# Tangshitao/Semi-supervised-Adaptive-Distillation

Hardware: AMD Instinct MI355X
Metric: images/sec (student+teacher fwd + student bwd) R50-FPN distill, 1/2/4/8 MI355X (higher is better)
Workload: dtype f32

## Files before the change

### include/ssad_kernels.h

```cpp
#ifndef SSAD_KERNELS_H_
#define SSAD_KERNELS_H_

#include <stddef.h>
#include <stdint.h>

#ifdef __cplusplus
extern "C" {
#endif

#define SSAD_API __attribute__((visibility("default")))

#define SSAD_E_BADARG (-1)
#define SSAD_E_WORKSPACE (-2)
#define SSAD_MAX_LEVELS 8
#define SSAD_MAX_CONV_PROBLEMS 24
#define SSAD_MAX_POWSUM_INPUTS 8

typedef void* ssad_stream_t;


typedef struct {
  float gamma;
  float alpha;
  float beta;
// ... 225 lines not shown
                         float* col, ssad_stream_t stream);
SSAD_API int ssad_im2col_batched(const float* x, int N, int C, int H, int W, int kernel, int stride,
                                 int pad, float* col, ssad_stream_t stream);
SSAD_API int ssad_col2im(const float* col, int C, int H, int W, int kh, int kw, int dil_h,
                         int dil_w, int pad_t, int pad_l, int pad_b, int pad_r, int stride_h,
                         int stride_w, float* x, ssad_stream_t stream);
SSAD_API int ssad_channel_sum(const float* dy, int N, int C, int HW, float* out, int accumulate,
                              ssad_stream_t stream);
SSAD_API int ssad_relu_grad_rowsum(const float* y, const float* dy, float* dx, float* rowsum, int N,
                                   int C, int HW, ssad_stream_t stream);
SSAD_API int ssad_conv1x1_bias_act(const float* x, const float* w, const float* bias,
                                   const float* residual, float* y, int N, int C, int P, int M,
                                   int relu, ssad_stream_t stream);
SSAD_API int ssad_conv1x1_bias_act2(const float* x, int C1, const float* x2, int C2, const float* w,
                                    const float* bias, const float* residual, float* y, int N, int P,
                                    int M, int relu, ssad_stream_t stream);
#define SSAD_GEMM_RELU 1
#define SSAD_GEMM_ACCUMULATE 8
typedef struct ssad_gemm_conv {
  const float* a;
  const float* x;
  float* y;
  const float* bias;
  const float* residual;
  const float* mask;
  int lda, N, K, P, M, flags;
} ssad_gemm_conv;
SSAD_API int ssad_conv1x1_gemm(const ssad_gemm_conv* desc_host, ssad_stream_t stream);
SSAD_API size_t ssad_conv1x1_gemm_split_workspace_bytes(const ssad_gemm_conv* desc_host);
SSAD_API int ssad_conv1x1_gemm_split(const ssad_gemm_conv* desc_host, void* workspace, size_t workspace_bytes,
                                     ssad_stream_t stream);
SSAD_API int ssad_conv1x1_gemm_split_amax(const ssad_gemm_conv* desc_host, const float* packed_a, const unsigned* x_amax,
                                          unsigned* y_amax_out, void* workspace, size_t workspace_bytes,
                                          ssad_stream_t stream);
typedef struct ssad_gemm_pack_entry {
  const float* a;
  float* dst;
  int lda, K, M;
} ssad_gemm_pack_entry;
SSAD_API size_t ssad_gemm_split_filter_floats(int K, int M);
SSAD_API int ssad_gemm_split_pack_filters(const ssad_gemm_pack_entry* entries_host, int n_entries, ssad_stream_t stream);
SSAD_API int ssad_conv_implicit_gemm(const ssad_gemm_conv* d, int C, int H, int W, int kernel, int stride, int pad,
                                     ssad_stream_t stream);
SSAD_API size_t ssad_conv_implicit_gemm_workspace_bytes(int N, int M, int C, int H, int W, int kernel, int stride,
                                                        int pad);
SSAD_API int ssad_conv_implicit_gemm_ws(const ssad_gemm_conv* d, int C, int H, int W, int kernel, int stride, int pad,
                                        void* workspace, size_t workspace_bytes, ssad_stream_t stream);
SSAD_API size_t ssad_conv_kxk_wgrad_workspace_bytes(int N, int C, int H, int W, int M, int kernel, int stride,
                                                    int pad);
SSAD_API int ssad_conv_kxk_wgrad(const float* x, const float* dy, int N, int C, int H, int W, int M, int kernel,
                                 int stride, int pad, float* dw, int accumulate, void* workspace,
                                 size_t workspace_bytes, ssad_stream_t stream);
SSAD_API size_t ssad_conv_kxk_dgrad_workspace_bytes(int N, int C, int H, int W, int M, int kernel, int stride,
                                                    int pad);
SSAD_API int ssad_conv_kxk_dgrad(const float* w, const float* dy, int N, int C, int H, int W, int M, int kernel,
                                 int stride, int pad, float* dx, const float* mask, int accumulate, void* workspace,
                                 size_t workspace_bytes, ssad_stream_t stream);
SSAD_API int ssad_transpose_filter(const float* w, int M, int K, int ldm, float* wt, ssad_stream_t stream);
#define SSAD_MAX_TRANSPOSE_ENTRIES 64
typedef struct ssad_transpose_entry {
  const float* w;
  float* wt;
  int M, K, ldm;
  int reserved;
} ssad_transpose_entry;
SSAD_API int ssad_transpose_filters(const ssad_transpose_entry* entries_host, int n_entries, ssad_stream_t stream);
// ... 146 lines not shown
```

### semi-supervised-adaptive-distillation_amd/csrc/kernels/gemm_split.hip

```cpp
#include <stdlib.h>

#include <mutex>

#include "split_common.h"

namespace {

using namespace ssad_split;

constexpr int PT = 128;
constexpr int MT = 256;
constexpr int HDR = 16;

__host__ __device__ constexpr int cdiv(int a, int b) { return (a + b - 1) / b; }

__global__ __launch_bounds__(kThreads) void gsplit_pack_a_kernel(const float* __restrict__ a, int lda, int K, int M,
                                                                 const unsigned* __restrict__ amax, float* __restrict__ dst) {
  const int KB = (K + 7) >> 3;
  const long long slots = (long long)KB * M;
  const float s = pow2f(15 - split_exponent(amax[0]));
  if (blockIdx.x == 0 && threadIdx.x < HDR) reinterpret_cast<unsigned*>(dst)[threadIdx.x] = threadIdx.x == 0 ? amax[0] : 0u;
  uint4* out = reinterpret_cast<uint4*>(dst + HDR);
  for (long long i = (long long)blockIdx.x * kThreads + threadIdx.x; i < slots; i += (long long)gridDim.x * kThreads) {
    const int m = (int)(i % M), kb = (int)(i / M);
    float v[8];
#pragma unroll
    for (int j = 0; j < 8; ++j) v[j] = kb * 8 + j < K ? a[(long long)(kb * 8 + j) * lda + m] : 0.0f;
    half8 hi, lo;
    split8(v, s, hi, lo);
    out[i] = __builtin_bit_cast(uint4, hi);
    out[slots + i] = __builtin_bit_cast(uint4, lo);
  }
}

struct GPackTable {
  ssad_gemm_pack_entry e[SSAD_MAX_PACK_ENTRIES];
  int count;
};
__global__ __launch_bounds__(kThreads) void gsplit_zero_kernel(const GPackTable t) {
  for (int i = (int)threadIdx.x; i < t.count * HDR; i += kThreads) reinterpret_cast<unsigned*>(t.e[i / HDR].dst)[i % HDR] = 0u;
}
__global__ __launch_bounds__(kThreads) void gsplit_amax_kernel(const GPackTable t) {
  const ssad_gemm_pack_entry& E = t.e[blockIdx.y];
// ... 9 lines not shown
    m = m > other ? m : other;
  }
  __shared__ unsigned red[kThreads / 64];
  if ((threadIdx.x & 63) == 0) red[threadIdx.x >> 6] = m;
  __syncthreads();
  if (threadIdx.x == 0) {
    for (int w = 1; w < kThreads / 64; ++w) m = m > red[w] ? m : red[w];
    if (m) atomicMax(reinterpret_cast<unsigned*>(E.dst), m);
  }
}
__global__ __launch_bounds__(kThreads) void gsplit_pack_multi_kernel(const GPackTable t) {
  const ssad_gemm_pack_entry& E = t.e[blockIdx.y];
  const int KB = (E.K + 7) >> 3;
  const long long slots = (long long)KB * E.M;
  const float s = pow2f(15 - split_exponent(reinterpret_cast<const unsigned*>(E.dst)[0]));
  uint4* out = reinterpret_cast<uint4*>(E.dst + HDR);
  for (long long i = (long long)blockIdx.x * kThreads + threadIdx.x; i < slots; i += (long long)gridDim.x * kThreads) {
    const int m = (int)(i % E.M), kb = (int)(i / E.M);
    float v[8];
#pragma unroll
    for (int j = 0; j < 8; ++j) v[j] = kb * 8 + j < E.K ? E.a[(long long)(kb * 8 + j) * E.lda + m] : 0.0f;
    half8 hi, lo;
    split8(v, s, hi, lo);
    out[i] = __builtin_bit_cast(uint4, hi);
    out[slots + i] = __builtin_bit_cast(uint4, lo);
  }
}

#ifndef GFLY_ABLATE
#define GFLY_ABLATE 0
#endif
constexpr int FKC = 32;
constexpr int FWG = 512;
constexpr int F_XP = (FKC / 8) * PT * 16;
constexpr int F_WP = (FKC / 8) * MT * 16;
constexpr int F_STAGE = 2 * F_XP + 2 * F_WP;
constexpr int F_LDS = 2 * F_STAGE;

struct FArgs {
  const float* x;
  const float* ap;
  float* y;
  const float* bias;
  const float* residual;
  const float* mask;
  const unsigned* amax;
  unsigned* amax_out;
  int N, K, P, M, relu, accumulate;
  int ptiles, mblocks, items;
};

__global__ __launch_bounds__(FWG, 1) void gemm_fly_kernel(const FArgs q) {
  extern __shared__ __attribute__((aligned(16))) char flds[];
  const int tid = threadIdx.x, lane = tid & 63;
  const int wave = __builtin_amdgcn_readfirstlane(tid >> 6);
  const int wm = wave & 3, wp = wave >> 2;
  const int j = lane & 31, h = lane >> 5;
  const int K = q.K, M = q.M, P = q.P;
  const int KB = (K + 7) >> 3;
  const int nchunks = (K + FKC - 1) / FKC;

  int n, p0, ocb;
  {
    const int it = (int)blockIdx.x;
    const int xcd = it & 7, seq = it >> 3;
    const int mb = seq % q.mblocks;
    const int t = (seq / q.mblocks) * 8 + xcd;
    if (t >= q.N * q.ptiles) return;
    n = t / q.ptiles;
    p0 = (t - n * q.ptiles) * PT;
    ocb = mb * MT;
  }
  const unsigned w_lo_off = (unsigned)((long long)KB * M * 16);
  const __amdgpu_buffer_rsrc_t xrs = uniform_rsrc(q.x, (unsigned)((long long)q.N * K * P * 4));
  const __amdgpu_buffer_rsrc_t wrs = uniform_rsrc(q.ap + HDR, 2u * w_lo_off);
  const float sx = pow2f(15 - split_exponent(q.amax[0]));

  float xv[8];
  f32x4 wv[4];
  const int fpx = tid & (PT - 1), fkg = tid >> 7;
  const int fco = tid & (MT - 1), fkq = tid >> 8;
  const unsigned xbase = p0 + fpx < P ? (unsigned)((((long long)n * K + 8 * fkg) * P + p0 + fpx) * 4) : kOob;
  const int P4 = P * 4;
  auto fetch = [&](int c) {
    const int soff = __builtin_amdgcn_readfirstlane(c * FKC * P4);
#pragma unroll
    for (int e = 0; e < 8; ++e)
      xv[e] = __builtin_bit_cast(float, __builtin_amdgcn_raw_buffer_load_b32(
          xrs, c * FKC + 8 * fkg + e < K ? xbase : kOob, soff + e * P4, 0));
#pragma unroll
    for (int i = 0; i < 2; ++i) {
      const int kb = c * (FKC / 8) + fkq + 2 * i;
      const unsigned vo = (kb < KB && ocb + fco < M) ? (unsigned)((kb * M + ocb + fco) * 16) : kOob;
      wv[2 * i] = __builtin_bit_cast(f32x4, __builtin_amdgcn_raw_buffer_load_b128(wrs, vo, 0, 0));
      wv[2 * i + 1] = __builtin_bit_cast(f32x4, __builtin_amdgcn_raw_buffer_load_b128(wrs, vo, (int)w_lo_off, 0));
    }
  };
  auto put = [&](char* stage) {
    half8 hi, lo;
    split8(xv, sx, hi, lo);
    char* px = stage + (fkg * PT + fpx) * 16;
    *reinterpret_cast<half8*>(px) = hi;
    *reinterpret_cast<half8*>(px + F_XP) = lo;
#pragma unroll
    for (int i = 0; i < 2; ++i) {
      char* pw = stage + 2 * F_XP + ((fkq + 2 * i) * MT + fco) * 16;
      *reinterpret_cast<f32x4*>(pw) = wv[2 * i];
      *reinterpret_cast<f32x4*>(pw + F_WP) = wv[2 * i + 1];
    }
  };

  float16v acc[2][2];
#pragma unroll
  for (int i = 0; i < 2; ++i)
#pragma unroll
    for (int tt = 0; tt < 2; ++tt)
#pragma unroll
      for (int r = 0; r < 16; ++r) acc[i][tt][r] = 0.0f;

  auto step = [&](const char* stage, int st) {
    half8 ah[2], al[2], bh[2], bl[2];
    const int kg = 2 * st + h;
#pragma unroll
    for (int i = 0; i < 2; ++i) {
      const char* pw = stage + 2 * F_XP + (kg * MT + wm * 64 + i * 32 + j) * 16;
      ah[i] = *reinterpret_cast<const half8*>(pw);
      al[i] = *reinterpret_cast<const half8*>(pw + F_WP);
      const char* px = stage + (kg * PT + wp * 64 + i * 32 + j) * 16;
      bh[i] = *reinterpret_cast<const half8*>(px);
      bl[i] = *reinterpret_cast<const half8*>(px + F_XP);
    }
#pragma unroll
    for (int pr = 0; pr < ((GFLY_ABLATE & 8) ? 0 : (GFLY_ABLATE & 4) ? 1 : 3); ++pr)
#pragma unroll
      for (int i = 0; i < 2; ++i)
#pragma unroll
        for (int tt = 0; tt < 2; ++tt)
          acc[i][tt] = __builtin_amdgcn_mfma_f32_32x32x16_f16(pr == 1 ? al[i] : ah[i], pr == 2 ? bl[tt] : bh[tt],
                                                              acc[i][tt], 0, 0, 0);
    if (GFLY_ABLATE & 8) {
#pragma unroll
      for (int i = 0; i < 2; ++i) { acc[i][0][0] += (float)ah[i][0] + (float)al[i][1]; acc[i][1][0] += (float)bh[i][0] + (float)bl[i][1]; }
    }
  };

  fetch(0);
  put(flds);
  fetch(1);
  __syncthreads();
  for (int c = 0; c < nchunks; ++c) {
    const char* stage = flds + (c & 1) * F_STAGE;
    char* other = flds + ((c & 1) ^ 1) * F_STAGE;
    __builtin_amdgcn_sched_barrier(0);
    step(stage, 0);
    if (!(GFLY_ABLATE & 2)) put(other);
    __builtin_amdgcn_sched_barrier(0);
    if (!(GFLY_ABLATE & 1)) fetch(c + 2);
    __builtin_amdgcn_sched_barrier(0);
    step(stage, 1);
    __syncthreads();
  }

  const int oc_w = ocb + wm * 64;
  unsigned pvo[2];
#pragma unroll
  for (int tt = 0; tt < 2; ++tt) {
    const int px = p0 + wp * 64 + 32 * tt + j;
    pvo[tt] = px < P ? (unsigned)((((long long)n * M + 4 * h) * P + px) * 4) : kOob;
  }
  const int e2 = split_exponent(q.amax[0]) + split_exponent(reinterpret_cast<const unsigned*>(q.ap)[0]) - 30;
  const bool one_scale = e2 >= -126 && e2 <= 127;
  const float sc1 = one_scale ? pow2f(e2) : pow2f(split_exponent(q.amax[0]) - 15);
  const float sc2 = one_scale ? 1.0f : pow2f(split_exponent(reinterpret_cast<const unsigned*>(q.ap)[0]) - 15);
  const unsigned ybytes = (unsigned)((long long)q.N * M * P * 4);
  const __amdgpu_buffer_rsrc_t yrs = uniform_rsrc(q.y, ybytes);
  const __amdgpu_buffer_rsrc_t rrs = uniform_rsrc(q.residual ? (const void*)q.residual : (const void*)q.y, q.residual ? ybytes : 0u);
  const __amdgpu_buffer_rsrc_t mrs = uniform_rsrc(q.mask ? (const void*)q.mask : (const void*)q.y, q.mask ? ybytes : 0u);
  const __amdgpu_buffer_rsrc_t brs = uniform_rsrc(q.bias ? (const void*)q.bias : (const void*)q.y, q.bias ? (unsigned)M * 4u : 0u);
  const bool relu = q.relu, has_res = q.residual != nullptr, has_mask = q.mask != nullptr, accum = q.accumulate;
  const bool ragged = (M & 7) != 0;
  unsigned ymax = 0;
#pragma unroll
  for (int i = 0; i < 2; ++i) {
    const int oc0 = oc_w + i * 32;
    float4 bq[4];
#pragma unroll
    for (int g = 0; g < 4; ++g)
      bq[g] = __builtin_bit_cast(float4, __builtin_amdgcn_raw_buffer_load_b128(brs, (unsigned)h * 16u, (oc0 + 8 * g) * 4, 0));
#pragma unroll
    for (int tt = 0; tt < 2; ++tt) {
      float rs[16], mk[16], old[16];
#pragma unroll
      for (int r = 0; r < 16; ++r) {
        const int ch = oc0 + 8 * (r >> 2) + (r & 3);
        const unsigned vo = (ch < M && (!ragged || ch + 4 * h < M)) ? pvo[tt] : kOob;
        rs[r] = has_res ? __builtin_bit_cast(float, __builtin_amdgcn_raw_buffer_load_b32(rrs, vo, ch * P4, 0)) : 0.0f;
        mk[r] = has_mask ? __builtin_bit_cast(float, __builtin_amdgcn_raw_buffer_load_b32(mrs, vo, ch * P4, 0)) : 1.0f;
        old[r] = accum ? __builtin_bit_cast(float, __builtin_amdgcn_raw_buffer_load_b32(yrs, vo, ch * P4, 0)) : 0.0f;
      }
#pragma unroll
      for (int g = 0; g < 4; ++g) {
        if (oc0 + 8 * g >= M) continue;
#pragma unroll
        for (int e = 0; e < 4; ++e) {
          const int r = 4 * g + e;
          float v = one_scale ? fmaf(acc[i][tt][r], sc1, bq[g][e]) : acc[i][tt][r] * sc1 * sc2 + bq[g][e];
          v += rs[r];
          if (relu) v = fmaxf(v, 0.0f);
          if (has_mask) v = mk[r] > 0.0f ? v : 0.0f;
          v += old[r];
          const unsigned vo = (!ragged || oc0 + 8 * g + 4 * h + e < M) ? pvo[tt] : kOob;
          __builtin_amdgcn_raw_buffer_store_b32(__builtin_bit_cast(unsigned, v), yrs, vo, (oc0 + 8 * g + e) * P4, 0);
          const unsigned av = __builtin_bit_cast(unsigned, v) & 0x7fffffffu;
          if (vo != kOob) ymax = ymax > av ? ymax : av;
        }
      }
    }
  }
  if (q.amax_out) {
#pragma unroll
    for (int o = 32; o > 0; o >>= 1) {
      const unsigned other = (unsigned)__shfl_xor((int)ymax, o, 64);
      ymax = ymax > other ? ymax : other;
    }
    __syncthreads();
    unsigned* red = reinterpret_cast<unsigned*>(flds);
    if (lane == 0) red[wave] = ymax;
    __syncthreads();
    if (tid == 0) {
      for (int w = 1; w < FWG / 64; ++w) ymax = ymax > red[w] ? ymax : red[w];
      if (ymax) atomicMax(q.amax_out, ymax);
    }
  }
}

constexpr int WT = 256;
constexpr int WPX = 32;
constexpr int W_PL = (WPX / 8) * WT * 16;
constexpr int W_STAGE = 4 * W_PL;
constexpr int W_LDS = 2 * W_STAGE;

struct WPArgs {
  const float* x;
  const float* dy;
  float* slabs;
  const unsigned* xa;
  const unsigned* da;
  int N, C, P, M;
  int mtiles, ctiles, shares, per_share, total, cpi;
  int xcd_runs;
};

__global__ __launch_bounds__(FWG, 1) void wpoint_split_kernel(const WPArgs q) {
  extern __shared__ __attribute__((aligned(16))) char wlds[];
  const int tid = threadIdx.x, lane = tid & 63;
  const int wave = __builtin_amdgcn_readfirstlane(tid >> 6);
  const int wm = wave & 1, wc = wave >> 1;
  const int j = lane & 31, h = lane >> 5;
  const int P = q.P;

  const int tiles = q.mtiles * q.ctiles;
  int share, tile;
  if (q.xcd_runs) {
// ... 119 lines not shown
__global__ __launch_bounds__(256) void wpoint_reduce_kernel(const float* __restrict__ slabs, int shares, int Mp, int Cp,
                                                            int M, int C, const unsigned* __restrict__ xa,
                                                            const unsigned* __restrict__ da,
                                                            float* __restrict__ dw, int accumulate) {
  const long long e = (long long)blockIdx.x * 256 + threadIdx.x;
  if (e >= (long long)M * C) return;
  const int m = (int)(e / C), c = (int)(e - (long long)m * C);
  const float* p = slabs + (long long)m * Cp + c;
  const long long stride = (long long)Mp * Cp;
  float s = 0.0f;
  for (int sh = 0; sh < shares; ++sh) s += p[sh * stride];
  s = (s * pow2f(split_exponent(xa[0]) - 15)) * pow2f(split_exponent(da[0]) - 15);
  dw[e] = accumulate ? dw[e] + s : s;
}

int wpoint_plan(int N, int C, int P, int M, WPArgs* a) {
  if (N <= 0 || C <= 0 || P <= 0 || M <= 0 || (P & 7)) return SSAD_E_BADARG;
  if ((long long)N * C * P * 4 >= (1LL << 31) || (long long)N * M * P * 4 >= (1LL << 31)) return SSAD_E_BADARG;
  a->N = N; a->C = C; a->P = P; a->M = M;
  a->mtiles = cdiv(M, WT); a->ctiles = cdiv(C, WT);
  a->cpi = cdiv(P, WPX);
  a->total = N * a->cpi;
  const int cus = ssad_cu_count(), tiles = a->mtiles * a->ctiles;
  int s = cus / tiles;
  if (s < 1) s = 1;
  if (s >= 8) s &= ~7;
  while (s > 1 && a->total / s < 4) --s;
  a->per_share = cdiv(a->total, s);
  a->shares = cdiv(a->total, a->per_share);
  a->xcd_runs = (a->shares % 8 == 0) ? a->shares / 8 : 0;
  return 0;
}

struct GPlan {
  size_t amax_off, a_off, total;
};
int make_plan(const ssad_gemm_conv* d, GPlan* p) {
  if (!d || d->N <= 0 || d->K <= 0 || d->P <= 0 || d->M <= 0 || d->lda < d->M) return SSAD_E_BADARG;
  const int KB = (d->K + 7) >> 3;
  const long long aslots = (long long)KB * d->M;
  if ((long long)d->N * d->K * d->P * 4 >= (1LL << 31) || (long long)d->N * d->M * d->P * 4 >= (1LL << 31) ||
      aslots * 32 >= (1LL << 31))
    return SSAD_E_BADARG;
  p->amax_off = 0;
  p->a_off = 256;
  p->total = p->a_off + (size_t)HDR * 4 + (size_t)aslots * 32;
  return 0;
}

}

extern "C" {

size_t ssad_conv1x1_gemm_split_workspace_bytes(const ssad_gemm_conv* d) {
  GPlan p;
  return make_plan(d, &p) ? 0 : p.total;
}

size_t ssad_gemm_split_filter_floats(int K, int M) {
  if (K <= 0 || M <= 0) return 0;
  return (size_t)HDR + (size_t)((K + 7) >> 3) * M * 8;
}

int ssad_gemm_split_pack_filters(const ssad_gemm_pack_entry* entries_host, int n_entries, ssad_stream_t stream_) {
  hipStream_t stream = (hipStream_t)stream_;
  if (!entries_host || n_entries < 0) return SSAD_E_BADARG;
  for (int base = 0; base < n_entries; base += SSAD_MAX_PACK_ENTRIES) {
    GPackTable t;
    const int cnt = n_entries - base < SSAD_MAX_PACK_ENTRIES ? n_entries - base : SSAD_MAX_PACK_ENTRIES;
    long long most = 0;
    for (int i = 0; i < cnt; ++i) {
      t.e[i] = entries_host[base + i];
      if (!t.e[i].a || !t.e[i].dst || t.e[i].K <= 0 || t.e[i].M <= 0 || t.e[i].lda < t.e[i].M) return SSAD_E_BADARG;
      const long long slots = (long long)((t.e[i].K + 7) >> 3) * t.e[i].M;
      if (slots > most) most = slots;
    }
    t.count = cnt;
    hipLaunchKernelGGL(gsplit_zero_kernel, dim3(1), dim3(kThreads), 0, stream, t);
    hipLaunchKernelGGL(gsplit_amax_kernel, dim3(64u, (unsigned)cnt), dim3(kThreads), 0, stream, t);
    long long bx = (most + kThreads - 1) / kThreads;
    if (bx > 256) bx = 256;
    hipLaunchKernelGGL(gsplit_pack_multi_kernel, dim3((unsigned)bx, (unsigned)cnt), dim3(kThreads), 0, stream, t);
  }
  return (int)hipGetLastError();
}

int ssad_conv1x1_gemm_split(const ssad_gemm_conv* d, void* workspace, size_t workspace_bytes, ssad_stream_t stream_) {
  return ssad_conv1x1_gemm_split_amax(d, nullptr, nullptr, nullptr, workspace, workspace_bytes, stream_);
}

int ssad_conv1x1_gemm_split_amax(const ssad_gemm_conv* d, const float* packed_a, const unsigned* x_amax,
                                 unsigned* y_amax_out, void* workspace, size_t workspace_bytes, ssad_stream_t stream_) {
  hipStream_t stream = (hipStream_t)stream_;
  GPlan p;
  const int rc = make_plan(d, &p);
  if (rc) return rc;
  if (!d->a || !d->x || !d->y) return SSAD_E_BADARG;
  if ((d->flags & SSAD_GEMM_ACCUMULATE) && (d->bias || d->residual)) return SSAD_E_BADARG;
  if (!workspace || workspace_bytes < p.total) return SSAD_E_WORKSPACE;
  char* ws = (char*)workspace;
  unsigned* amax = (unsigned*)(ws + p.amax_off);
  float* apk = (float*)(ws + p.a_off);
  const int KB = (d->K + 7) >> 3;
  AmaxTable at;
  for (int l = 0; l < kMaxLv; ++l) { at.x[l] = nullptr; at.n[l] = 0; at.block_start[l] = 0; }
  at.count = 2;
  at.amax = amax;
  at.x[0] = d->x; at.n[0] = (long long)d->N * d->K * d->P;
  at.x[1] = d->a; at.n[1] = (long long)d->K * d->lda;
  int blocks = 0;
  for (int l = 0; l < 2; ++l) {
    at.block_start[l] = blocks;
    long long nb = (at.n[l] / 4 + kThreads * 32 - 1) / (kThreads * 32);
    blocks += (int)(nb < 1 ? 1 : nb > 512 ? 512 : nb);
  }
  for (int l = 2; l <= kMaxLv; ++l) at.block_start[l] = blocks;
  if (x_amax && packed_a) {
  } else {
    if (x_amax) { at.n[0] = 0; }
    if (packed_a) { at.n[1] = 0; }
    (void)hipMemsetAsync(amax, 0, 256, stream);
    hipLaunchKernelGGL(split_absmax_kernel, dim3((unsigned)blocks), dim3(kThreads), 0, stream, at);
    if (!packed_a) {
      long long bx = ((long long)KB * d->M + kThreads - 1) / kThreads;
      if (bx > 1024) bx = 1024;
      hipLaunchKernelGGL(gsplit_pack_a_kernel, dim3((unsigned)bx), dim3(kThreads), 0, stream, d->a, d->lda, d->K, d->M,
                         (const unsigned*)(amax + 1), apk);
    }
  }
  FArgs f;
  f.x = d->x; f.ap = packed_a ? packed_a : apk; f.y = d->y; f.bias = d->bias; f.residual = d->residual; f.mask = d->mask;
  f.amax = x_amax ? x_amax : amax;
  f.amax_out = y_amax_out;
  f.N = d->N; f.K = d->K; f.P = d->P; f.M = d->M;
  f.relu = (d->flags & SSAD_GEMM_RELU) ? 1 : 0;
  f.accumulate = (d->flags & SSAD_GEMM_ACCUMULATE) ? 1 : 0;
  f.ptiles = cdiv(d->P, PT);
  f.mblocks = cdiv(d->M, MT);
  const long long tiles = (long long)d->N * f.ptiles;
  if (tiles * f.mblocks >= (1LL << 30)) return SSAD_E_BADARG;
  f.items = (int)(cdiv((int)tiles, 8) * 8 * f.mblocks);
  static std::once_flag lds_once;
  std::call_once(lds_once, [&] {
    (void)hipFuncSetAttribute((const void*)gemm_fly_kernel, hipFuncAttributeMaxDynamicSharedMemorySize, F_LDS);
  });
  hipLaunchKernelGGL(gemm_fly_kernel, dim3((unsigned)f.items), dim3(FWG), F_LDS, stream, f);
  return (int)hipGetLastError();
}

int ssad_split_absmax(const float* x, long long n, unsigned* word, ssad_stream_t stream_) {
  if (!x || !word || n <= 0) return SSAD_E_BADARG;
  AmaxTable at;
  for (int l = 0; l < kMaxLv; ++l) { at.x[l] = nullptr; at.n[l] = 0; at.block_start[l] = 0; }
  at.count = 1;
  at.amax = word;
  at.x[0] = x; at.n[0] = n;
  long long nb = (n / 4 + kThreads * 32 - 1) / (kThreads * 32);
  const int blocks = (int)(nb < 1 ? 1 : nb > 512 ? 512 : nb);
  for (int l = 1; l <= kMaxLv; ++l) at.block_start[l] = blocks;
  hipLaunchKernelGGL(split_absmax_kernel, dim3((unsigned)blocks), dim3(kThreads), 0, (hipStream_t)stream_, at);
  return (int)hipGetLastError();
}

size_t ssad_conv1x1_wgrad_split_workspace_bytes(int N, int C, int P, int M) {
  WPArgs a;
  if (wpoint_plan(N, C, P, M, &a)) return 0;
  return 256 + sizeof(float) * (size_t)a.shares * a.mtiles * WT * a.ctiles * WT;
}

int ssad_conv1x1_wgrad_split(const float* x, const float* dy, int N, int C, int P, int M, float* dw, int accumulate,
                             void* workspace, size_t workspace_bytes, ssad_stream_t stream_) {
  return ssad_conv1x1_wgrad_split_amax(x, dy, N, C, P, M, dw, accumulate, workspace, workspace_bytes, nullptr, nullptr,
                                       stream_);
}

int ssad_conv1x1_wgrad_split_amax(const float* x, const float* dy, int N, int C, int P, int M, float* dw, int accumulate,
                                  void* workspace, size_t workspace_bytes, const unsigned* x_amax,
                                  const unsigned* dy_amax, ssad_stream_t stream_) {
  hipStream_t stream = (hipStream_t)stream_;
  if ((x_amax == nullptr) != (dy_amax == nullptr)) return SSAD_E_BADARG;
// ... 41 lines not shown
```

### semi-supervised-adaptive-distillation_amd/kernels.py

```python
import ctypes as C
import os

import torch

_HERE = os.path.dirname(os.path.abspath(__file__))
LIB_NAME = "libcaffe2_detectron_ops_hip.so"
LIB_PATH = os.path.join(_HERE, LIB_NAME)

MAX_LEVELS = 8
CONV_RELU = 1
CONV_MASK_AUX = 2
CONV_SIGMOID = 4
CONV_SPLIT_TAIL = 8


class KernelError(RuntimeError):
    pass


class DistillParams(C.Structure):
    _fields_ = [("gamma", C.c_float), ("alpha", C.c_float), ("beta", C.c_float),
                ("num_classes", C.c_int), ("ignored_label", C.c_int),
                ("scale", C.c_float)]

# ... 150 lines not shown
    L.ssad_conv_wino_pack_filter.argtypes = [vp, i32, i32, vp, vp, vp]
    L.ssad_conv3x3_forward_wino.argtypes = [C.POINTER(ConvLevel), i32, vp, vp, i32, i32, i32, vp]
    L.ssad_conv3x3_forward_wino24.argtypes = [C.POINTER(ConvLevel), i32, vp, vp, i32, i32, i32, vp]
    L.ssad_conv_wino24_filter_floats.restype = sz
    L.ssad_conv_wino24_filter_floats.argtypes = [i32, i32]
    L.ssad_conv_wino24_pack_filters.argtypes = [C.POINTER(PackEntry), i32, vp]
    L.ssad_conv_split_filter_floats.restype = sz
    L.ssad_conv_split_filter_floats.argtypes = [i32, i32]
    L.ssad_conv_split_pack_filters.argtypes = [C.POINTER(PackEntry), i32, vp]
    L.ssad_conv3x3_split_workspace_bytes.restype = sz
    L.ssad_conv3x3_split_workspace_bytes.argtypes = [C.POINTER(ConvLevel), i32, i32]
    L.ssad_conv3x3_forward_split.argtypes = [C.POINTER(ConvLevel), i32, vp, vp, i32, i32, i32, vp, sz, vp, vp, vp]
    L.ssad_conv3x3_forward_wino_launches.argtypes = [C.POINTER(ConvLevel), i32]
    L.ssad_conv3x3_forward_wino_launches_for.argtypes = [C.POINTER(ConvLevel), i32, i32, i32, i32]
    L.ssad_conv_wino_split_tail.argtypes = [i32]
    L.ssad_conv3x3_wgrad_workspace_bytes.restype = sz
    L.ssad_conv3x3_wgrad_workspace_bytes.argtypes = [C.POINTER(ConvLevel), i32, i32, i32]
    L.ssad_conv3x3_wgrad.argtypes = [C.POINTER(ConvLevel), i32, vp, vp, i32, i32, i32, vp, sz, vp]
    L.ssad_conv3x3_wgrad_split_workspace_bytes.restype = sz
    L.ssad_conv3x3_wgrad_split_workspace_bytes.argtypes = [C.POINTER(ConvLevel), i32, i32, i32]
    L.ssad_conv3x3_wgrad_split.argtypes = [C.POINTER(ConvLevel), i32, vp, vp, i32, i32, i32, vp, sz, vp]
    L.ssad_conv1x1_gemm.argtypes = [C.POINTER(GemmConv), vp]
    L.ssad_conv1x1_gemm_split_workspace_bytes.restype = sz
    L.ssad_conv1x1_gemm_split_workspace_bytes.argtypes = [C.POINTER(GemmConv)]
    L.ssad_conv1x1_gemm_split.argtypes = [C.POINTER(GemmConv), vp, sz, vp]
    L.ssad_transpose_filter.argtypes = [vp, i32, i32, i32, vp, vp]
    L.ssad_conv1x1_wgrad_workspace_bytes.restype = sz
    L.ssad_conv1x1_wgrad_workspace_bytes.argtypes = [i32, i32, i32, i32]
    L.ssad_conv1x1_wgrad.argtypes = [vp, vp, i32, i32, i32, i32, vp, i32, vp, sz, vp]
    L.ssad_gemm_split_filter_floats.restype = sz
    L.ssad_gemm_split_filter_floats.argtypes = [i32, i32]
    L.ssad_gemm_split_pack_filters.argtypes = [C.POINTER(GemmPackEntry), i32, vp]
    L.ssad_conv1x1_gemm_split_amax.argtypes = [vp, vp, vp, vp, vp, sz, vp]
    L.ssad_split_absmax.argtypes = [vp, C.c_longlong, vp, vp]
    L.ssad_split_absmax_levels.argtypes = [C.POINTER(ConvLevel), i32, i32, i32, vp, vp]
    L.ssad_conv3x3_wgrad_split_amax.argtypes = [C.POINTER(ConvLevel), i32, vp, vp, i32, i32, i32, vp, sz, vp, vp, vp]
    L.ssad_conv1x1_wgrad_split_amax.argtypes = [vp, vp, i32, i32, i32, i32, vp, i32, vp, sz, vp, vp, vp]
    L.ssad_conv1x1_wgrad_split_workspace_bytes.restype = sz
    L.ssad_conv1x1_wgrad_split_workspace_bytes.argtypes = [i32, i32, i32, i32]
    L.ssad_conv1x1_wgrad_split.argtypes = [vp, vp, i32, i32, i32, i32, vp, i32, vp, sz, vp]
    L.ssad_subsample.argtypes = [vp, i32, i32, i32, i32, i32, vp, vp]
    L.ssad_subsample_grad.argtypes = [vp, i32, i32, i32, i32, i32, i32, vp, vp]
    L.ssad_conv_implicit_gemm.argtypes = [C.POINTER(GemmConv), i32, i32, i32, i32, i32, i32, vp]
    L.ssad_transpose_filters.argtypes = [C.POINTER(TransposeEntry), i32, vp]
    L.ssad_f16_pack_filters.argtypes = [C.POINTER(F16PackEntry), i32, vp]
    L.ssad_conv_implicit_gemm_workspace_bytes.restype = sz
    L.ssad_conv_implicit_gemm_workspace_bytes.argtypes = [i32] * 8
    L.ssad_conv_implicit_gemm_ws.argtypes = [C.POINTER(GemmConv), i32, i32, i32, i32, i32, i32, vp, sz, vp]
    L.ssad_conv_kxk_wgrad_workspace_bytes.restype = sz
    L.ssad_conv_kxk_wgrad_workspace_bytes.argtypes = [i32] * 8
    L.ssad_conv_kxk_wgrad.argtypes = [vp, vp, i32, i32, i32, i32, i32, i32, i32, i32, vp, i32, vp, sz, vp]
    L.ssad_conv_kxk_dgrad_workspace_bytes.restype = sz
    L.ssad_conv_kxk_dgrad_workspace_bytes.argtypes = [i32] * 8
    L.ssad_conv_kxk_dgrad.argtypes = [vp, vp, i32, i32, i32, i32, i32, i32, i32, i32, vp, vp, i32, vp, sz, vp]
    L.ssad_grouped_conv3x3_forward.argtypes = [vp, vp, vp, i32, i32, i32, i32, i32, i32, i32, vp, vp]
    L.ssad_grouped_conv3x3_filter_floats.argtypes = [i32, i32]
    L.ssad_grouped_conv3x3_filter_floats.restype = C.c_longlong
    L.ssad_grouped_conv3x3_pack_filter.argtypes = [vp, i32, i32, vp, vp]
    L.ssad_conv1x1_f16.argtypes = [C.POINTER(PwF16), vp]
    L.ssad_pw_f16_filter_halves.restype = sz
    L.ssad_pw_f16_filter_halves.argtypes = [i32, i32]
    L.ssad_pw_f16_pack_filter.argtypes = [vp, i32, i32, vp, vp, vp]
    L.ssad_conv1x1_wgrad_f16_workspace_bytes.restype = sz
    L.ssad_conv1x1_wgrad_f16_workspace_bytes.argtypes = [i32, i32, i32, i32, i32]
    L.ssad_conv1x1_wgrad_f16.argtypes = [vp, vp, i32, i32, i32, i32, i32, i32, f32, vp, vp, vp, vp, sz, vp]
    L.ssad_f16_elementwise.argtypes = [i32, vp, vp, vp, i32, i32, i32, i32, i32, i32, vp]
# ... 612 lines not shown
            arr[i].packed = p["packed"].data_ptr()
            arr[i].bias = p["bias"].data_ptr() if p.get("bias") is not None else None
            i += 1
    flags = ((CONV_RELU if relu else 0) | (CONV_SIGMOID if sigmoid else 0)
             | (CONV_MASK_AUX if masked[0] else 0) | (F16_OUT_NCHW_F32 if out_nchw_f32 else 0))
    _check(lib().ssad_conv3x3_forward_f16_levels(arr, n, None, None, Cin, Cout, flags, _stream()),
           "conv3x3_forward_f16_multi")


def conv3x3_wgrad_f16(xbs, dybs, Cin, Cout, *, scale=1.0, dW=None, db=None, bias_grad=True):
    if dW is None:
        dW = torch.empty((Cout, Cin, 3, 3), dtype=torch.float32, device="cuda")
    if db is None and bias_grad:
        db = torch.empty((Cout,), dtype=torch.float32, device="cuda")
    L = lib()
    n = len(xbs)
    arr = (F16WgradLevel * n)()
    for i, (xb, dyb) in enumerate(zip(xbs, dybs)):
        N, CB, H, W, _ = xb.shape
        assert xb.dtype == torch.float16 and dyb.dtype == torch.float16
        assert xb.is_contiguous() and dyb.is_contiguous()
        assert CB == (Cin + 7) // 8 and dyb.shape == (N, (Cout + 7) // 8, H, W, 8)
        arr[i].x, arr[i].dy, arr[i].N, arr[i].H, arr[i].W = xb.data_ptr(), dyb.data_ptr(), N, H, W
    nbytes = L.ssad_conv3x3_wgrad_f16_levels_workspace_bytes(arr, n, Cin, Cout)
    ws = _workspace(nbytes, "wgrad_f16")
    _check(L.ssad_conv3x3_wgrad_f16_levels(arr, n, Cin, Cout, 0, float(scale), _ptr(dW), _ptr(db), _ptr(ws),
                                           nbytes, _stream()), "conv3x3_wgrad_f16_levels")
    return dW, db



GEMM_RELU = 1
GEMM_ACCUMULATE = 8


def transpose_filter(w, out=None):
    M, Kc = w.shape[0], w.shape[1]
    w2 = _f32c(w.reshape(M, Kc), "w")
    ldm = (M + 3) // 4 * 4
    wt = out if out is not None else torch.empty((Kc, ldm), dtype=torch.float32, device="cuda")
    _check(lib().ssad_transpose_filter(_ptr(w2), M, Kc, ldm, _ptr(wt), _stream()), "transpose_filter")
    return wt


def gemm_conv_desc(a, lda, x, y, K, M, bias=None, residual=None, mask=None, relu=False, accumulate=False):
    N = x.shape[0]
    P = x.numel() // max(N * K, 1)
    return GemmConv(a.data_ptr(), x.data_ptr(), y.data_ptr(), bias.data_ptr() if bias is not None else 0,
                    residual.data_ptr() if residual is not None else 0,
                    mask.data_ptr() if mask is not None else 0, lda, N, K, P, M,
                    (GEMM_RELU if relu else 0) | (GEMM_ACCUMULATE if accumulate else 0))


def _run_gemm(d, what, split):
    L = lib()
    if not split:
        _check(L.ssad_conv1x1_gemm(C.byref(d), _stream()), what)
        return
    need = L.ssad_conv1x1_gemm_split_workspace_bytes(C.byref(d))
    ws = torch.empty(max(need, 16), dtype=torch.uint8, device="cuda")
    _check(L.ssad_conv1x1_gemm_split(C.byref(d), _ptr(ws), ws.numel(), _stream()), what + " (split)")


def split_absmax(x, word=None):
    _f32c(x, "x")
    if word is None:
# ... 161 lines not shown
```

Before: 239.0.

## Add 4-wave direct-weight GEMM variant and specialize epilogue at compile time

Templates the split-precision 1x1 GEMM kernel on pixel tile and wave count. It adds a 4-wave form that loads weights straight from global memory into registers instead of staging them in LDS, so two workgroups can share a CU's LDS. The epilogue is also specialized at compile time for the residual, mask and accumulate cases, and ragged-edge bounds checks become branchless. Auto selection still returns the 8-wave form, so the new path runs only when called explicitly; the default path gains only the specialized epilogue.

```diff
diff --git a/include/ssad_kernels.h b/include/ssad_kernels.h
--- a/include/ssad_kernels.h
+++ b/include/ssad_kernels.h
@@ -281,6 +281,12 @@
                                      ssad_stream_t stream);
 SSAD_API int ssad_conv1x1_gemm_split_amax(const ssad_gemm_conv* desc_host, const float* packed_a, const unsigned* x_amax,
                                           unsigned* y_amax_out, void* workspace, size_t workspace_bytes,
+                                          ssad_stream_t stream);
+#define SSAD_GEMM_FLY_AUTO 0
+#define SSAD_GEMM_FLY_8WAVE 1
+#define SSAD_GEMM_FLY_4WAVE 2
+SSAD_API int ssad_conv1x1_gemm_split_form(const ssad_gemm_conv* desc_host, const float* packed_a, const unsigned* x_amax,
+                                          unsigned* y_amax_out, void* workspace, size_t workspace_bytes, int form,
                                           ssad_stream_t stream);
 typedef struct ssad_gemm_pack_entry {
   const float* a;
diff --git a/semi-supervised-adaptive-distillation_amd/csrc/kernels/gemm_split.hip b/semi-supervised-adaptive-distillation_amd/csrc/kernels/gemm_split.hip
--- a/semi-supervised-adaptive-distillation_amd/csrc/kernels/gemm_split.hip
+++ b/semi-supervised-adaptive-distillation_amd/csrc/kernels/gemm_split.hip
@@ -1,6 +1,7 @@
 #include <stdlib.h>
 
 #include <mutex>
+#include <type_traits>
 
 #include "split_common.h"
 
@@ -8,7 +9,6 @@
 
 using namespace ssad_split;
 
-constexpr int PT = 128;
 constexpr int MT = 256;
 constexpr int HDR = 16;
 
@@ -84,10 +84,7 @@
 #endif
 constexpr int FKC = 32;
 constexpr int FWG = 512;
-constexpr int F_XP = (FKC / 8) * PT * 16;
 constexpr int F_WP = (FKC / 8) * MT * 16;
-constexpr int F_STAGE = 2 * F_XP + 2 * F_WP;
-constexpr int F_LDS = 2 * F_STAGE;
 
 struct FArgs {
   const float* x;
@@ -102,7 +99,21 @@
   int ptiles, mblocks, items;
 };
 
-__global__ __launch_bounds__(FWG, 1) void gemm_fly_kernel(const FArgs q) {
+template <int PT_, int WAVES>
+struct FlyShape {
+  static_assert(WAVES == 4 * (PT_ / 64) && (PT_ == 64 || PT_ == 128), "waves are 4 (channel) x PT_ / 64 (pixel)");
+  static constexpr bool kDirect = WAVES == 4;
+  static constexpr int kThreadsWg = WAVES * 64;
+  static constexpr int kXP = (FKC / 8) * PT_ * 16;
+  static constexpr int kStage = 2 * kXP + (kDirect ? 0 : 2 * F_WP);
+  static constexpr int kLds = 2 * kStage;
+  static_assert(!kDirect || 2 * kLds <= 160 * 1024, "two workgroups of the 4-wave form share a CU's LDS");
+};
+
+template <int PT_, int WAVES>
+__global__ __launch_bounds__(WAVES * 64, WAVES == 8 ? 1 : 2) void gemm_fly_kernel(const FArgs q) {
+  using S = FlyShape<PT_, WAVES>;
+  constexpr int F_XP = S::kXP, F_STAGE = S::kStage;
   extern __shared__ __attribute__((aligned(16))) char flds[];
   const int tid = threadIdx.x, lane = tid & 63;
   const int wave = __builtin_amdgcn_readfirstlane(tid >> 6);
@@ -120,7 +131,7 @@
     const int t = (seq / q.mblocks) * 8 + xcd;
     if (t >= q.N * q.ptiles) return;
     n = t / q.ptiles;
-    p0 = (t - n * q.ptiles) * PT;
+    p0 = (t - n * q.ptiles) * PT_;
     ocb = mb * MT;
   }
   const unsigned w_lo_off = (unsigned)((long long)KB * M * 16);
@@ -129,59 +140,43 @@
   const float sx = pow2f(15 - split_exponent(q.amax[0]));
 
   float xv[8];
-  f32x4 wv[4];
-  const int fpx = tid & (PT - 1), fkg = tid >> 7;
+  const int fpx = tid & (PT_ - 1), fkg = tid / PT_;
   const int fco = tid & (MT - 1), fkq = tid >> 8;
   const unsigned xbase = p0 + fpx < P ? (unsigned)((((long long)n * K + 8 * fkg) * P + p0 + fpx) * 4) : kOob;
   const int P4 = P * 4;
-  auto fetch = [&](int c) {
+  auto fetch_x = [&](int c) {
     const int soff = __builtin_amdgcn_readfirstlane(c * FKC * P4);
 #pragma unroll
     for (int e = 0; e < 8; ++e)
       xv[e] = __builtin_bit_cast(float, __builtin_amdgcn_raw_buffer_load_b32(
           xrs, c * FKC + 8 * fkg + e < K ? xbase : kOob, soff + e * P4, 0));
-#pragma unroll
-    for (int i = 0; i < 2; ++i) {
-      const int kb = c * (FKC / 8) + fkq + 2 * i;
-      const unsigned vo = (kb < KB && ocb + fco < M) ? (unsigned)((kb * M + ocb + fco) * 16) : kOob;
-      wv[2 * i] = __builtin_bit_cast(f32x4, __builtin_amdgcn_raw_buffer_load_b128(wrs, vo, 0, 0));
-      wv[2 * i + 1] = __builtin_bit_cast(f32x4, __builtin_amdgcn_raw_buffer_load_b128(wrs, vo, (int)w_lo_off, 0));
-    }
   };
-  auto put = [&](char* stage) {
+  auto put_x = [&](char* stage) {
     half8 hi, lo;
     split8(xv, sx, hi, lo);
-    char* px = stage + (fkg * PT + fpx) * 16;
+    char* px = stage + (fkg * PT_ + fpx) * 16;
     *reinterpret_cast<half8*>(px) = hi;
     *reinterpret_cast<half8*>(px + F_XP) = lo;
+  };
+  auto read_x = [&](const char* stage, int st, half8 (&bh)[2], half8 (&bl)[2]) {
+    const int kg = 2 * st + h;
 #pragma unroll
     for (int i = 0; i < 2; ++i) {
-      char* pw = stage + 2 * F_XP + ((fkq + 2 * i) * MT + fco) * 16;
-      *reinterpret_cast<f32x4*>(pw) = wv[2 * i];
-      *reinterpret_cast<f32x4*>(pw + F_WP) = wv[2 * i + 1];
-    }
-  };
-
-  float16v acc[2][2];
-#pragma unroll
-  for (int i = 0; i < 2; ++i)
-#pragma unroll
-    for (int tt = 0; tt < 2; ++tt)
-#pragma unroll
-      for (int r = 0; r < 16; ++r) acc[i][tt][r] = 0.0f;
-
-  auto step = [&](const char* stage, int st) {
-    half8 ah[2], al[2], bh[2], bl[2];
-    const int kg = 2 * st + h;
-#pragma unroll
-    for (int i = 0; i < 2; ++i) {
-      const char* pw = stage + 2 * F_XP + (kg * MT + wm * 64 + i * 32 + j) * 16;
-      ah[i] = *reinterpret_cast<const half8*>(pw);
-      al[i] = *reinterpret_cast<const half8*>(pw + F_WP);
-      const char* px = stage + (kg * PT + wp * 64 + i * 32 + j) * 16;
+      const char* px = stage + (kg * PT_ + wp * 64 + i * 32 + j) * 16;
       bh[i] = *reinterpret_cast<const half8*>(px);
       bl[i] = *reinterpret_cast<const half8*>(px + F_XP);
     }
+  };
+
+  float16v acc[2][2];
+#pragma unroll
+  for (int i = 0; i < 2; ++i)
+#pragma unroll
+    for (int tt = 0; tt < 2; ++tt)
+#pragma unroll
+      for (int r = 0; r < 16; ++r) acc[i][tt][r] = 0.0f;
+
+  auto mfmas = [&](const half8 (&ah)[2], const half8 (&al)[2], const half8 (&bh)[2], const half8 (&bl)[2]) {
 #pragma unroll
     for (int pr = 0; pr < ((GFLY_ABLATE & 8) ? 0 : (GFLY_ABLATE & 4) ? 1 : 3); ++pr)
 #pragma unroll
@@ -196,21 +191,103 @@
     }
   };
 
-  fetch(0);
-  put(flds);
-  fetch(1);
-  __syncthreads();
-  for (int c = 0; c < nchunks; ++c) {
-    const char* stage = flds + (c & 1) * F_STAGE;
-    char* other = flds + ((c & 1) ^ 1) * F_STAGE;
-    __builtin_amdgcn_sched_barrier(0);
-    step(stage, 0);
-    if (!(GFLY_ABLATE & 2)) put(other);
-    __builtin_amdgcn_sched_barrier(0);
-    if (!(GFLY_ABLATE & 1)) fetch(c + 2);
-    __builtin_amdgcn_sched_barrier(0);
-    step(stage, 1);
+  if constexpr (S::kDirect) {
+    typedef half8 WSet[2][2][2];
+    const unsigned wrow = (unsigned)(ocb + wm * 64 + j);
+    auto fetch_w = [&](int c, WSet& w) {
+#pragma unroll
+      for (int st = 0; st < 2; ++st) {
+        const int kb = c * (FKC / 8) + 2 * st + h;
+#pragma unroll
+        for (int i = 0; i < 2; ++i) {
+          const unsigned row = wrow + 32u * i;
+          const unsigned vo = (kb < KB && row < (unsigned)M) ? ((unsigned)kb * (unsigned)M + row) * 16u : kOob;
+          w[st][i][0] = __builtin_bit_cast(half8, __builtin_amdgcn_raw_buffer_load_b128(wrs, vo, 0, 0));
+          w[st][i][1] = __builtin_bit_cast(half8, __builtin_amdgcn_raw_buffer_load_b128(wrs, vo, (int)w_lo_off, 0));
+        }
+      }
+    };
+    auto step = [&](const char* stage, int st, const WSet& w) {
+      half8 ah[2], al[2], bh[2], bl[2];
+      read_x(stage, st, bh, bl);
+#pragma unroll
+      for (int i = 0; i < 2; ++i) { ah[i] = w[st][i][0]; al[i] = w[st][i][1]; }
+      mfmas(ah, al, bh, bl);
+    };
+    auto chunk = [&](int c, const WSet& cur, WSet& nxt) {
+      const char* stage = flds + (c & 1) * F_STAGE;
+      char* other = flds + ((c & 1) ^ 1) * F_STAGE;
+      __builtin_amdgcn_sched_barrier(0);
+      if (!(GFLY_ABLATE & 1)) fetch_w(c + 1, nxt);
+      __builtin_amdgcn_sched_barrier(0);
+      step(stage, 0, cur);
+      if (!(GFLY_ABLATE & 2)) put_x(other);
+      __builtin_amdgcn_sched_barrier(0);
+      if (!(GFLY_ABLATE & 1)) fetch_x(c + 2);
+      __builtin_amdgcn_sched_barrier(0);
+      step(stage, 1, cur);
+      __syncthreads();
+    };
+    WSet w0, w1;
+    fetch_x(0);
+    fetch_w(0, w0);
+    if (GFLY_ABLATE & 1) fetch_w(1, w1);
+    put_x(flds);
+    fetch_x(1);
     __syncthreads();
+    for (int c = 0; c < nchunks; c += 2) {
+      chunk(c, w0, w1);
+      if (c + 1 < nchunks) chunk(c + 1, w1, w0);
+    }
+  } else {
+    f32x4 wv[4];
+    auto fetch = [&](int c) {
+      fetch_x(c);
+#pragma unroll
+      for (int i = 0; i < 2; ++i) {
+        const int kb = c * (FKC / 8) + fkq + 2 * i;
+        const unsigned vo = (kb < KB && ocb + fco < M) ? (unsigned)((kb * M + ocb + fco) * 16) : kOob;
+        wv[2 * i] = __builtin_bit_cast(f32x4, __builtin_amdgcn_raw_buffer_load_b128(wrs, vo, 0, 0));
+        wv[2 * i + 1] = __builtin_bit_cast(f32x4, __builtin_amdgcn_raw_buffer_load_b128(wrs, vo, (int)w_lo_off, 0));
+      }
+    };
+    auto put = [&](char* stage) {
+      put_x(stage);
+#pragma unroll
+      for (int i = 0; i < 2; ++i) {
+        char* pw = stage + 2 * F_XP + ((fkq + 2 * i) * MT + fco) * 16;
+        *reinterpret_cast<f32x4*>(pw) = wv[2 * i];
+        *reinterpret_cast<f32x4*>(pw + F_WP) = wv[2 * i + 1];
+      }
+    };
+    auto step = [&](const char* stage, int st) {
+      half8 ah[2], al[2], bh[2], bl[2];
+      const int kg = 2 * st + h;
+#pragma unroll
+      for (int i = 0; i < 2; ++i) {
+        const char* pw = stage + 2 * F_XP + (kg * MT + wm * 64 + i * 32 + j) * 16;
+        ah[i] = *reinterpret_cast<const half8*>(pw);
+        al[i] = *reinterpret_cast<const half8*>(pw + F_WP);
+      }
+      read_x(stage, st, bh, bl);
+      mfmas(ah, al, bh, bl);
+    };
+    fetch(0);
+    put(flds);
+    fetch(1);
+    __syncthreads();
+    for (int c = 0; c < nchunks; ++c) {
+      const char* stage = flds + (c & 1) * F_STAGE;
+      char* other = flds + ((c & 1) ^ 1) * F_STAGE;
+      __builtin_amdgcn_sched_barrier(0);
+      step(stage, 0);
+      if (!(GFLY_ABLATE & 2)) put(other);
+      __builtin_amdgcn_sched_barrier(0);
+      if (!(GFLY_ABLATE & 1)) fetch(c + 2);
+      __builtin_amdgcn_sched_barrier(0);
+      step(stage, 1);
+      __syncthreads();
+    }
   }
 
   const int oc_w = ocb + wm * 64;
@@ -229,45 +306,59 @@
   const __amdgpu_buffer_rsrc_t rrs = uniform_rsrc(q.residual ? (const void*)q.residual : (const void*)q.y, q.residual ? ybytes : 0u);
   const __amdgpu_buffer_rsrc_t mrs = uniform_rsrc(q.mask ? (const void*)q.mask : (const void*)q.y, q.mask ? ybytes : 0u);
   const __amdgpu_buffer_rsrc_t brs = uniform_rsrc(q.bias ? (const void*)q.bias : (const void*)q.y, q.bias ? (unsigned)M * 4u : 0u);
-  const bool relu = q.relu, has_res = q.residual != nullptr, has_mask = q.mask != nullptr, accum = q.accumulate;
-  const bool ragged = (M & 7) != 0;
+  const bool relu = q.relu;
+  const int mrem = M - 4 * h;
   unsigned ymax = 0;
-#pragma unroll
-  for (int i = 0; i < 2; ++i) {
-    const int oc0 = oc_w + i * 32;
-    float4 bq[4];
-#pragma unroll
-    for (int g = 0; g < 4; ++g)
-      bq[g] = __builtin_bit_cast(float4, __builtin_amdgcn_raw_buffer_load_b128(brs, (unsigned)h * 16u, (oc0 + 8 * g) * 4, 0));
-#pragma unroll
-    for (int tt = 0; tt < 2; ++tt) {
-      float rs[16], mk[16], old[16];
-#pragma unroll
-      for (int r = 0; r < 16; ++r) {
-        const int ch = oc0 + 8 * (r >> 2) + (r & 3);
-        const unsigned vo = (ch < M && (!ragged || ch + 4 * h < M)) ? pvo[tt] : kOob;
-        rs[r] = has_res ? __builtin_bit_cast(float, __builtin_amdgcn_raw_buffer_load_b32(rrs, vo, ch * P4, 0)) : 0.0f;
-        mk[r] = has_mask ? __builtin_bit_cast(float, __builtin_amdgcn_raw_buffer_load_b32(mrs, vo, ch * P4, 0)) : 1.0f;
-        old[r] = accum ? __builtin_bit_cast(float, __builtin_amdgcn_raw_buffer_load_b32(yrs, vo, ch * P4, 0)) : 0.0f;
-      }
-#pragma unroll
-      for (int g = 0; g < 4; ++g) {
-        if (oc0 + 8 * g >= M) continue;
-#pragma unroll
-        for (int e = 0; e < 4; ++e) {
-          const int r = 4 * g + e;
-          float v = one_scale ? fmaf(acc[i][tt][r], sc1, bq[g][e]) : acc[i][tt][r] * sc1 * sc2 + bq[g][e];
-          v += rs[r];
-          if (relu) v = fmaxf(v, 0.0f);
-          if (has_mask) v = mk[r] > 0.0f ? v : 0.0f;
-          v += old[r];
-          const unsigned vo = (!ragged || oc0 + 8 * g + 4 * h + e < M) ? pvo[tt] : kOob;
-          __builtin_amdgcn_raw_buffer_store_b32(__builtin_bit_cast(unsigned, v), yrs, vo, (oc0 + 8 * g + e) * P4, 0);
-          const unsigned av = __builtin_bit_cast(unsigned, v) & 0x7fffffffu;
-          if (vo != kOob) ymax = ymax > av ? ymax : av;
+  auto epilogue = [&](auto res_c, auto mask_c, auto acc_c) {
+    constexpr bool has_res = decltype(res_c)::value, has_mask = decltype(mask_c)::value, accum = decltype(acc_c)::value;
+#pragma unroll
+    for (int i = 0; i < 2; ++i) {
+      const int oc0 = oc_w + i * 32;
+      float4 bq[4];
+#pragma unroll
+      for (int g = 0; g < 4; ++g)
+        bq[g] = __builtin_bit_cast(float4, __builtin_amdgcn_raw_buffer_load_b128(brs, (unsigned)h * 16u, (oc0 + 8 * g) * 4, 0));
+#pragma unroll
+      for (int tt = 0; tt < 2; ++tt) {
+        float rs[16], mk[16], old[16];
+        unsigned vos[16];
+#pragma unroll
+        for (int r = 0; r < 16; ++r) {
+          const int ch = oc0 + 8 * (r >> 2) + (r & 3);
+          const unsigned gone = (unsigned)(mrem - 1 - ch) & kOob;
+          const unsigned vo = pvo[tt] > gone ? pvo[tt] : gone;
+          vos[r] = vo;
+          rs[r] = has_res ? __builtin_bit_cast(float, __builtin_amdgcn_raw_buffer_load_b32(rrs, vo, ch * P4, 0)) : 0.0f;
+          mk[r] = has_mask ? __builtin_bit_cast(float, __builtin_amdgcn_raw_buffer_load_b32(mrs, vo, ch * P4, 0)) : 1.0f;
+          old[r] = accum ? __builtin_bit_cast(float, __builtin_amdgcn_raw_buffer_load_b32(yrs, vo, ch * P4, 0)) : 0.0f;
+        }
+#pragma unroll
+        for (int g = 0; g < 4; ++g) {
+          if (oc0 + 8 * g >= M) continue;
+#pragma unroll
+          for (int e = 0; e < 4; ++e) {
+            const int r = 4 * g + e;
+            float v = one_scale ? fmaf(acc[i][tt][r], sc1, bq[g][e]) : acc[i][tt][r] * sc1 * sc2 + bq[g][e];
+            v += rs[r];
+            if (relu) v = fmaxf(v, 0.0f);
+            if (has_mask) v = mk[r] > 0.0f ? v : 0.0f;
+            v += old[r];
+            __builtin_amdgcn_raw_buffer_store_b32(__builtin_bit_cast(unsigned, v), yrs, vos[r], (oc0 + 8 * g + e) * P4, 0);
+            const unsigned av = __builtin_bit_cast(unsigned, v) & 0x7fffffffu;
+            if (vos[r] != kOob) ymax = ymax > av ? ymax : av;
+          }
         }
       }
     }
+  };
+  using Yes = std::true_type;
+  using No = std::false_type;
+  if (q.accumulate) {
+    if (q.mask) epilogue(No{}, Yes{}, Yes{}); else epilogue(No{}, No{}, Yes{});
+  } else if (q.residual) {
+    if (q.mask) epilogue(Yes{}, Yes{}, No{}); else epilogue(Yes{}, No{}, No{});
+  } else {
+    if (q.mask) epilogue(No{}, Yes{}, No{}); else epilogue(No{}, No{}, No{});
   }
   if (q.amax_out) {
 #pragma unroll
@@ -280,7 +371,7 @@
     if (lane == 0) red[wave] = ymax;
     __syncthreads();
     if (tid == 0) {
-      for (int w = 1; w < FWG / 64; ++w) ymax = ymax > red[w] ? ymax : red[w];
+      for (int w = 1; w < WAVES; ++w) ymax = ymax > red[w] ? ymax : red[w];
       if (ymax) atomicMax(q.amax_out, ymax);
     }
   }
@@ -466,6 +557,28 @@
   return 0;
 }
 
+int fly_form(int K, int M, int P) {
+  (void)K; (void)M; (void)P;
+  return SSAD_GEMM_FLY_8WAVE;
+}
+
+template <int PT_, int WAVES>
+int launch_fly(FArgs& f, hipStream_t stream) {
+  using S = FlyShape<PT_, WAVES>;
+  f.ptiles = cdiv(f.P, PT_);
+  const long long tiles = (long long)f.N * f.ptiles;
+  if (tiles * f.mblocks >= (1LL << 30)) return SSAD_E_BADARG;
+  f.items = (int)(cdiv((int)tiles, 8) * 8 * f.mblocks);
+  if (S::kLds > 64 * 1024) {
+    static std::once_flag lds_once;
+    std::call_once(lds_once, [&] {
+      (void)hipFuncSetAttribute((const void*)gemm_fly_kernel<PT_, WAVES>, hipFuncAttributeMaxDynamicSharedMemorySize, S::kLds);
+    });
+  }
+  hipLaunchKernelGGL((gemm_fly_kernel<PT_, WAVES>), dim3((unsigned)f.items), dim3(S::kThreadsWg), S::kLds, stream, f);
+  return (int)hipGetLastError();
+}
+
 struct GPlan {
   size_t amax_off, a_off, total;
 };
@@ -525,6 +638,13 @@
 
 int ssad_conv1x1_gemm_split_amax(const ssad_gemm_conv* d, const float* packed_a, const unsigned* x_amax,
                                  unsigned* y_amax_out, void* workspace, size_t workspace_bytes, ssad_stream_t stream_) {
+  return ssad_conv1x1_gemm_split_form(d, packed_a, x_amax, y_amax_out, workspace, workspace_bytes, SSAD_GEMM_FLY_AUTO,
+                                      stream_);
+}
+
+int ssad_conv1x1_gemm_split_form(const ssad_gemm_conv* d, const float* packed_a, const unsigned* x_amax,
+                                 unsigned* y_amax_out, void* workspace, size_t workspace_bytes, int form,
+                                 ssad_stream_t stream_) {
   hipStream_t stream = (hipStream_t)stream_;
   GPlan p;
   const int rc = make_plan(d, &p);
@@ -569,17 +689,11 @@
   f.N = d->N; f.K = d->K; f.P = d->P; f.M = d->M;
   f.relu = (d->flags & SSAD_GEMM_RELU) ? 1 : 0;
   f.accumulate = (d->flags & SSAD_GEMM_ACCUMULATE) ? 1 : 0;
-  f.ptiles = cdiv(d->P, PT);
   f.mblocks = cdiv(d->M, MT);
-  const long long tiles = (long long)d->N * f.ptiles;
-  if (tiles * f.mblocks >= (1LL << 30)) return SSAD_E_BADARG;
-  f.items = (int)(cdiv((int)tiles, 8) * 8 * f.mblocks);
-  static std::once_flag lds_once;
-  std::call_once(lds_once, [&] {
-    (void)hipFuncSetAttribute((const void*)gemm_fly_kernel, hipFuncAttributeMaxDynamicSharedMemorySize, F_LDS);
-  });
-  hipLaunchKernelGGL(gemm_fly_kernel, dim3((unsigned)f.items), dim3(FWG), F_LDS, stream, f);
-  return (int)hipGetLastError();
+  if (form == SSAD_GEMM_FLY_AUTO) form = fly_form(d->K, d->M, d->P);
+  if (form == SSAD_GEMM_FLY_4WAVE) return launch_fly<64, 4>(f, stream);
+  if (form == SSAD_GEMM_FLY_8WAVE) return launch_fly<128, 8>(f, stream);
+  return SSAD_E_BADARG;
 }
 
 int ssad_split_absmax(const float* x, long long n, unsigned* word, ssad_stream_t stream_) {
diff --git a/semi-supervised-adaptive-distillation_amd/kernels.py b/semi-supervised-adaptive-distillation_amd/kernels.py
--- a/semi-supervised-adaptive-distillation_amd/kernels.py
+++ b/semi-supervised-adaptive-distillation_amd/kernels.py
@@ -206,6 +206,7 @@
     L.ssad_gemm_split_filter_floats.argtypes = [i32, i32]
     L.ssad_gemm_split_pack_filters.argtypes = [C.POINTER(GemmPackEntry), i32, vp]
     L.ssad_conv1x1_gemm_split_amax.argtypes = [vp, vp, vp, vp, vp, sz, vp]
+    L.ssad_conv1x1_gemm_split_form.argtypes = [vp, vp, vp, vp, vp, sz, i32, vp]
     L.ssad_split_absmax.argtypes = [vp, C.c_longlong, vp, vp]
     L.ssad_split_absmax_levels.argtypes = [C.POINTER(ConvLevel), i32, i32, i32, vp, vp]
     L.ssad_conv3x3_wgrad_split_amax.argtypes = [C.POINTER(ConvLevel), i32, vp, vp, i32, i32, i32, vp, sz, vp, vp, vp]
@@ -884,6 +885,7 @@
 
 GEMM_RELU = 1
 GEMM_ACCUMULATE = 8
+GEMM_FLY_AUTO, GEMM_FLY_8WAVE, GEMM_FLY_4WAVE = 0, 1, 2
 
 
 def transpose_filter(w, out=None):
```

Measured after the change: 240.6 (median of 4 runs). No clear change (+0.7%).
